# google-research/weatherbench2

Hardware: AMD Instinct MI355X
Metric: grid-point-evals/sec (721x1440x13) (higher is better)
Workload: dtype f32 (elementwise) + f64 (sums); 1 GPU; BASELINE configs[1]: 721x1440x13 f32, deterministic MSE+RMSE+MAE+Bias+ACC, 13 predefined slice regions, running init-time mean; pool_units=48, regions=13, rows_per_chunk=32, step=one wb2_det_suite_step call (K1 + K2 + time accumulate), parallelism=init-time shards x1, 1 all-reduce of [sum,count], launcher=single process

## Files before the change

### include/wb2hip.h

```cpp
#ifndef WB2HIP_H_
#define WB2HIP_H_

#include <stdint.h>

#ifdef __cplusplus
extern "C" {
#endif

#define WB2_VERSION 1

#define WB2_F32 0
#define WB2_F64 1

#define WB2_MODE_DET 0
#define WB2_MODE_DET_ACC 1
#define WB2_MODE_WIND 2

#define WB2_MODE_ENS 3

#define WB2_MODE_GAUSS 4
#define WB2_MODE_GAUSS_THR 5
#define WB2_MODE_SEEPS 7
#define WB2_MODE_ENS_THR 6

// ... 180 lines not shown

int wb2_ens_combine(int skipna, const double* partials, int64_t n_outer,
                    int32_t n_chunk, int32_t nwf, int32_t n_seg,
                    const int32_t* seg_eoff, int32_t n_ts,
                    const int32_t* band_chunk0, int32_t n_band,
                    const double* coef_band, const double* coef_seg,
                    const int32_t* region_wf, const double* region_wsum,
                    int32_t n_region, double* sums, double* metrics,
                    void* stream);

int wb2_time_accumulate(const double* values, int64_t n_lead, int64_t n_time,
                        int64_t n_tail, int skipna, double* sum, double* count,
                        void* stream);

int wb2_time_accumulate_scatter(int dtype, const void* values, int64_t n_lead,
                                int64_t n_time, int64_t n_tail, int skipna,
                                const int64_t* dst, double* sum, double* count,
                                void* stream);
int wb2_time_accumulate_runs(int dtype, const void* values, int64_t n_lead,
                             int64_t n_time, int64_t n_tail, int skipna,
                             const int64_t* dst, int64_t run, double* sum,
                             double* count, void* stream);

typedef struct wb2_plan_tables {
  int32_t n_row, n_col;
  int32_t n_chunk, n_ctile;
  int32_t n_seg, n_ts;
  int32_t n_band, n_region;
  const double* w_row;
  const double* w_col;
  const void* wfield;
  int32_t wfield_dtype;
  int32_t reserved;
  const double* aux;
  double scalar;
  const int32_t* chunk_row0;
  const int32_t* chunk_nrow;
  const int32_t* seg_col0;
  const int32_t* seg_eoff;
  const int32_t* band_chunk0;
  const double* coef_band;
  const double* coef_seg;
  const int32_t* region_wf;
  const double* region_wsum;
} wb2_plan_tables;

int wb2_det_suite_step(const wb2_plan_tables* plan, int mode, int dtype,
                       int skipna, const void* const* in,
                       const int64_t* const* slab, int aligned16,
                       int64_t n_outer, double* partials, double* metrics,
                       int64_t acc_lead, int64_t acc_time, int64_t acc_tail,
                       int acc_skipna, const int64_t* dst, double* sum,
                       double* count, void* stream);

int wb2_det_wind_suite_step(const wb2_plan_tables* plan, int mode, int dtype,
                            int skipna, const void* const* in,
                            const int64_t* const* slab, int aligned16,
                            int64_t n_outer, int64_t n_pair, double* partials,
                            double* wind_partials, double* metrics,
                            double* wind_metrics, void* stream);

int wb2_gather_accumulate(const double* arena, const int32_t* src,
                          const uint8_t* round32, int64_t n_out, int64_t n_time,
                          int skipna, const int64_t* sum_addr,
                          const int64_t* count_addr, void* stream);

int wb2_gather_accumulate_rows(const double* arena, const int32_t* src,
                               const uint8_t* round32, int64_t n_out,
                               int64_t n_time, int skipna,
                               const int64_t* sum_addr,
                               const int64_t* count_addr, const int64_t* rows,
                               const int32_t* sel, const int64_t* rsz8,
                               void* stream);

int wb2_program_create(void** program);
int wb2_program_destroy(void* program);
int wb2_program_add_launch(void* program, const wb2_plan_tables* plan, int mode,
                           int dtype, int skipna, int32_t n_in, int64_t n_outer,
                           int64_t n_pair, const int32_t* slot,
                           const int64_t* rel, double* partials,
                           double* wind_partials, int64_t arena_offset,
                           int side_stream);
int wb2_program_add_ens_launch(void* program, const wb2_plan_tables* plan,
                               int dtype, int skipna, int32_t n_member,
                               int64_t member_stride, int64_t n_outer,
                               const int32_t* slot, const int64_t* rel,
                               double* partials, int64_t arena_offset);
int wb2_program_add_gather(void* program, int32_t input, int64_t first,
                           int64_t count, int32_t source, int64_t step_bytes,
                           int32_t value_offset, const int32_t* cell,
                           const int64_t* base);
int wb2_program_add_sink(void* program, const int32_t* src,
                         const uint8_t* round32, int64_t n_out, int64_t n_time,
                         int skipna, const int32_t* sel, const int64_t* rsz8,
                         int64_t max_rows);
int wb2_program_finalize(void* program, double* arena, int32_t n_ptrs,
                         int32_t n_values);
int wb2_program_replay(void* program, const int64_t* ptrs, int32_t n_ptrs,
                       const int64_t* values, int32_t n_values,
                       const int64_t* sink_args, const int64_t* rows,
                       int32_t n_rows, void* stream);
int wb2_program_stats(void* program, double* seconds, int64_t* replays);

int wb2_energy_layout(int32_t n_member, int skipna, int has_wfield,
                      int32_t* block, int32_t* n_block, int32_t* n_slot);
int wb2_energy_score(int dtype, int skipna, const void* ens,
// ... 162 lines not shown
```

### weatherbench2_amd/_lib.py

```python
from __future__ import annotations

import ctypes
import os

import torch

from weatherbench2_amd import build as _build

WB2_F32, WB2_F64 = 0, 1
MODE_DET, MODE_DET_ACC, MODE_WIND, MODE_ENS, MODE_GAUSS = 0, 1, 2, 3, 4
MODE_GAUSS_THR, MODE_ENS_THR, MODE_SEEPS = 5, 6, 7
GENERIC_KQ = {MODE_GAUSS: 2, MODE_GAUSS_THR: 3, MODE_ENS_THR: 4,
              MODE_SEEPS: 1}
NMETRIC = 5
NMETRIC_ENS = 8
METRIC_INDEX = {'mse': 0, 'rmse': 1, 'mae': 2, 'bias': 3, 'acc': 4}
ENS_METRIC_INDEX = {'crps': 0, 'crps_spread': 1, 'crps_skill': 2,
                    'ensemble_mean_mse': 3, 'ensemble_mean_rmse': 4,
                    'ensemble_variance': 5, 'ensemble_stddev': 6,
                    'debiased_ensemble_mean_mse': 7}

_c = ctypes
_vp, _i32, _i64, _int = _c.c_void_p, _c.c_int32, _c.c_int64, _c.c_int
_u64 = _c.c_uint64



class PlanTables(_c.Structure):
  _fields_ = [
      ('n_row', _i32), ('n_col', _i32), ('n_chunk', _i32), ('n_ctile', _i32),
      ('n_seg', _i32), ('n_ts', _i32), ('n_band', _i32), ('n_region', _i32),
      ('w_row', _vp), ('w_col', _vp), ('wfield', _vp),
      ('wfield_dtype', _i32), ('reserved', _i32), ('aux', _vp),
      ('scalar', _c.c_double), ('chunk_row0', _vp), ('chunk_nrow', _vp),
      ('seg_col0', _vp), ('seg_eoff', _vp), ('band_chunk0', _vp),
      ('coef_band', _vp), ('coef_seg', _vp), ('region_wf', _vp),
      ('region_wsum', _vp)]


_SIGNATURES = {
    'wb2_version': (_int, []),
    'wb2_last_error': (_c.c_char_p, []),
    'wb2_num_slots': (_int, [_int, _int]),
    'wb2_tile_cols': (_int, [_int, _int, _int]),
    'wb2_tile_cols_ex': (_int, [_int, _int, _int, _int, _int, _int]),
    'wb2_stream_partials': (_int, [
        _int, _int, _int, _c.POINTER(_vp), _c.POINTER(_vp), _i64, _i32, _i32,
        _vp, _vp, _vp, _vp, _vp, _i32, _i32, _vp, _vp, _i32, _i32, _vp, _vp]),
    'wb2_stream_partials_ex': (_int, [
        _int, _int, _int, _c.POINTER(_vp), _c.POINTER(_vp), _i64, _i32, _i32,
        _vp, _vp, _vp, _int, _vp, _c.c_double, _vp, _vp, _i32, _i32, _vp, _vp,
        _i32, _i32, _vp, _vp]),
    'wb2_stream_partials_addr': (_int, [
        _int, _int, _int, _c.POINTER(_vp), _int, _i64, _i32, _i32,
        _vp, _vp, _vp, _int, _vp, _c.c_double, _vp, _vp, _i32, _i32, _vp, _vp,
        _i32, _i32, _vp, _vp]),
    'wb2_pairs_supported': (_int, [_int, _int, _int, _int, _int, _int]),
    'wb2_stream_partials_pairs': (_int, [
        _int, _int, _int, _c.POINTER(_vp), _c.POINTER(_vp), _int, _i64, _i64,
        _i32, _i32, _vp, _vp, _vp, _int, _vp, _vp, _i32, _i32, _vp, _vp, _i32,
        _i32, _vp, _vp, _vp]),
    'wb2_det_wind_suite_step': (_int, [
        _c.POINTER(PlanTables), _int, _int, _int, _c.POINTER(_vp),
        _c.POINTER(_vp), _int, _i64, _i64, _vp, _vp, _vp, _vp, _vp]),
    'wb2_det_combine': (_int, [
        _int, _int, _vp, _i64, _i32, _i32, _i32, _vp, _i32, _vp, _i32, _vp,
        _vp, _vp, _vp, _i32, _vp, _vp, _vp]),
    'wb2_det_suite_step': (_int, [
        _c.POINTER(PlanTables), _int, _int, _int, _c.POINTER(_vp),
        _c.POINTER(_vp), _int, _i64, _vp, _vp, _i64, _i64, _i64, _int, _vp,
        _vp, _vp, _vp]),
    'wb2_gather_accumulate': (_int, [_vp, _vp, _vp, _i64, _i64, _int, _vp, _vp,
                                     _vp]),
    'wb2_gather_accumulate_rows': (_int, [_vp, _vp, _vp, _i64, _i64, _int,
                                          _vp, _vp, _vp, _vp, _vp, _vp]),
    'wb2_program_create': (_int, [_c.POINTER(_vp)]),
    'wb2_program_destroy': (_int, [_vp]),
    'wb2_program_add_launch': (_int, [
        _vp, _c.POINTER(PlanTables), _int, _int, _int, _i32, _i64, _i64, _vp,
        _vp, _vp, _vp, _i64, _int]),
    'wb2_program_add_ens_launch': (_int, [
        _vp, _c.POINTER(PlanTables), _int, _int, _i32, _i64, _i64, _vp, _vp,
        _vp, _i64]),
    'wb2_program_add_gather': (_int, [_vp, _i32, _i64, _i64, _i32, _i64, _i32,
                                      _vp, _vp]),
    'wb2_program_add_sink': (_int, [_vp, _vp, _vp, _i64, _i64, _int, _vp, _vp,
                                    _i64]),
    'wb2_program_finalize': (_int, [_vp, _vp, _i32, _i32]),
    'wb2_program_replay': (_int, [_vp, _vp, _i32, _vp, _i32, _vp, _vp, _i32,
                                  _vp]),
    'wb2_program_stats': (_int, [_vp, _c.POINTER(_c.c_double),
                                 _c.POINTER(_i64)]),
    'wb2_energy_layout': (_int, [_i32, _int, _int, _c.POINTER(_i32),
                                 _c.POINTER(_i32), _c.POINTER(_i32)]),
    'wb2_energy_score': (_int, [
        _int, _int, _vp, _vp, _vp, _vp, _i32, _i64, _i64,
        _c.POINTER(PlanTables), _vp, _vp, _vp, _vp]),
    'wb2_time_accumulate': (_int, [_vp, _i64, _i64, _i64, _int, _vp, _vp,
                                   _vp]),
    'wb2_time_accumulate_scatter': (_int, [_int, _vp, _i64, _i64, _i64, _int,
                                           _vp, _vp, _vp, _vp]),
    'wb2_time_accumulate_runs': (_int, [_int, _vp, _i64, _i64, _i64, _int,
                                        _vp, _i64, _vp, _vp, _vp]),
    'wb2_ens_partials': (_int, [
        _int, _int, _vp, _vp, _vp, _vp, _i32, _i64, _i64, _i32, _i32, _vp, _vp,
        _vp, _vp, _vp, _i32, _i32, _vp, _vp, _i32, _i32, _vp, _vp]),
    'wb2_ens_partials_maps': (_int, [
        _int, _int, _vp, _vp, _vp, _vp, _i32, _i64, _i64, _i32, _i32, _vp, _vp,
        _vp, _vp, _vp, _i32, _i32, _vp, _vp, _i32, _i32, _vp, _vp, _vp]),
    'wb2_ens_partials_addr': (_int, [
        _int, _int, _vp, _vp, _i32, _i64, _i64, _i32, _i32, _vp, _vp, _vp, _vp,
        _vp, _i32, _i32, _vp, _vp, _i32, _i32, _vp, _vp]),
    'wb2_ens_partials_gather': (_int, [
        _int, _int, _vp, _vp, _vp, _i32, _i64, _i32, _i32, _vp, _vp, _vp, _vp,
        _vp, _i32, _i32, _vp, _vp, _i32, _i32, _vp, _vp, _vp]),
    'wb2_ens_threshold_partials': (_int, [
        _int, _int, _vp, _vp, _vp, _vp, _vp, _vp, _i32, _i64, _i64, _i32, _i32,
        _vp, _vp, _vp, _vp, _vp, _i32, _i32, _vp, _vp, _i32, _i32, _vp, _vp]),
    'wb2_ens_threshold_maps': (_int, [
        _int, _int, _vp, _vp, _vp, _vp, _vp, _vp, _i32, _i64, _i64, _i64, _vp,
        _vp]),
    'wb2_seeps_map': (_int, [_int, _c.POINTER(_vp), _c.POINTER(_vp), _i64, _i64,
                             _vp, _c.c_double, _vp, _vp]),
    'wb2_seeps_map_addr': (_int, [_int, _c.POINTER(_vp), _i64, _i64, _vp,
# ... 134 lines not shown
```

### weatherbench2_amd/csrc/stream_reduce.hip

```cpp

#include "common.hpp"
#include "trace.hpp"
#include "reduce_common.hpp"
#include "gauss_math.hpp"
#include "wb2hip.h"

#include <atomic>
#include <type_traits>

namespace wb2 {
namespace {

constexpr int kMaxIn = 4;

struct StreamParams {
  const void* in[kMaxIn];
  const long long* slab[kMaxIn];
  const double* w_row;
  const double* w_col;
  const void* wfield;
  const double* aux;
  double scalar;
  const int* chunk_row0;
  const int* chunk_nrow;
// ... 752 lines not shown
  } else {
#pragma clang loop unroll(disable)
    for (; r + U <= nrow; r += U, ++it)
      batch_v(std::integral_constant<int, U>{}, r, it & 1);
#pragma clang loop unroll(disable)
    for (; r < nrow; ++r, ++it)
      batch_v(std::integral_constant<int, 1>{}, r, it & 1);
  }

  if (p.w_col) {
#pragma unroll
    for (int e = 0; e < VEC; ++e) {
      const double wc = p.w_col[colb + e];
#pragma unroll
      for (int w = 0; w < NWF; ++w) {
#pragma unroll
        for (int k = 0; k < KD; ++k) acc[w][e][k] *= wc;
#pragma unroll
        for (int k = 0; k < KW; ++k) accw[w][e][k] *= wc;
      }
    }
  }
  fold_tile_to_segs<NWF, VEC, KD>(
      acc, lane, tile, colb, col0, p.n_col, p.seg_col0, p.seg_eoff, p.n_seg,
      p.n_ts,
      p.partials + (o * p.n_chunk + chunk) * (long long)(NWF * p.n_ts * KD));
  if (role == 1)
    fold_tile_to_segs<NWF, VEC, KW>(
        accw, lane, tile, colb, col0, p.n_col, p.seg_col0, p.seg_eoff, p.n_seg,
        p.n_ts,
        pp.wind_partials +
            (pair * p.n_chunk + chunk) * (long long)(NWF * p.n_ts * KW));
}

struct CombineParams {
  const double* partials;
  const int* seg_eoff;
  const int* band_chunk0;
  const double* coef_band;
  const double* coef_seg;
  const int* region_wf;
  const double* region_wsum;
  double* sums;
  double* metrics;
  long long n_outer;
  int n_chunk, nwf, n_seg, n_ts, n_band, n_region, K, mode, skipna;
  int group;
};

__device__ __forceinline__ double nan_if_zero(double d) {
  return d != 0.0 ? d : __builtin_nan("");
}

__device__ __forceinline__ void det_combine_body(const CombineParams& p,
                                                 const long long o,
                                                 double* lds) {
  const int K = p.K;
  const int cell = p.nwf * p.n_seg * K;
  double* bandsum = lds;
  double* rsum = lds + p.n_band * cell;
  const int tid = threadIdx.x;
  double* cseg = rsum + p.n_region * K * (1 + p.n_band);
  double* cband = cseg + p.n_region * p.n_seg;
  for (int i = tid; i < p.n_region * p.n_seg; i += blockDim.x)
    cseg[i] = p.coef_seg[i];
  for (int i = tid; i < p.n_region * p.n_band; i += blockDim.x)
    cband[i] = p.coef_band[i];
  const long long chunk_stride = (long long)p.nwf * p.n_ts * K;
  const double* part = p.partials + o * p.n_chunk * chunk_stride;

  if (p.group > 1) {
    const int G = p.group;
    for (int idx = tid; idx < p.n_band * cell * G; idx += blockDim.x) {
      const int ci = idx / G, g = idx - ci * G;
      const int b = ci / cell, j = ci - b * cell;
      const int w = j / (p.n_seg * K), sk = j - w * (p.n_seg * K);
      const int s = sk / K, k = sk - s * K;
      const int e0 = p.seg_eoff[s], ne = p.seg_eoff[s + 1] - e0;
      const int c0 = p.band_chunk0[b], n = (p.band_chunk0[b + 1] - c0) * ne;
      const double* base = part + ((long long)w * p.n_ts) * K + k +
                           c0 * chunk_stride + (long long)e0 * K;
      int c = g / ne, e = g - c * ne;
      const int dq = G / ne, dr = G - dq * ne;
      auto next = [&]() {
        const double* r = base + c * chunk_stride + (long long)e * K;
        c += dq;
        e += dr;
        if (e >= ne) {
          e -= ne;
          ++c;
        }
        return r;
      };
      double v = 0.0;
      int i = g;
      for (; i + 7 * G < n; i += 8 * G) {
        double t[8];
#pragma unroll
        for (int u = 0; u < 8; ++u) t[u] = *next();
#pragma unroll
        for (int u = 0; u < 8; ++u) v += t[u];
      }
      for (; i < n; i += G) v += *next();
      for (int off = G >> 1; off > 0; off >>= 1) v += __shfl_xor(v, off, kWave);
      if (g == 0) bandsum[ci] = v;
    }
  } else
  for (int idx = tid; idx < p.n_band * cell; idx += blockDim.x) {
    const int b = idx / cell, j = idx - b * cell;
    const int w = j / (p.n_seg * K), sk = j - w * (p.n_seg * K);
    const int s = sk / K, k = sk - s * K;
    const int e0 = p.seg_eoff[s], ne = p.seg_eoff[s + 1] - e0;
    const int c0 = p.band_chunk0[b], n = (p.band_chunk0[b + 1] - c0) * ne;
    const double* base = part + ((long long)w * p.n_ts) * K + k;
    const double* q = base + c0 * chunk_stride + (long long)e0 * K;
    const long long wrap = chunk_stride - (long long)ne * K;
    int e = 0;
    auto next = [&]() {
      const double* r = q;
      q += K;
      if (++e == ne) {
        e = 0;
        q += wrap;
      }
      return r;
    };
    double v = 0.0;
    int i = 0;
    for (; i + 32 <= n; i += 32) {
      double t[32];
#pragma unroll
      for (int u = 0; u < 32; ++u) t[u] = *next();
#pragma unroll
      for (int u = 0; u < 32; ++u) v += t[u];
    }
    for (; i + 16 <= n; i += 16) {
      double t[16];
#pragma unroll
      for (int u = 0; u < 16; ++u) t[u] = *next();
#pragma unroll
      for (int u = 0; u < 16; ++u) v += t[u];
    }
    for (; i + 4 <= n; i += 4) {
      double t[4];
#pragma unroll
      for (int u = 0; u < 4; ++u) t[u] = *next();
#pragma unroll
      for (int u = 0; u < 4; ++u) v += t[u];
    }
    for (; i < n; ++i) v += *next();
    bandsum[idx] = v;
  }
  __syncthreads();
  double* rb = rsum + p.n_region * K;
  for (int idx = tid; idx < p.n_region * p.n_band * K; idx += blockDim.x) {
    const int r = idx / (p.n_band * K), bk = idx - r * (p.n_band * K);
    const int b = bk / K, k = bk - b * K;
    const int wf = p.region_wf[r];
    const double cb = cband[r * p.n_band + b];
    double v = 0.0;
    if (cb != 0.0) {
      const double* row = bandsum + ((b * p.nwf + wf) * p.n_seg) * K + k;
      for (int s = 0; s < p.n_seg; ++s) {
        const double cs = cseg[r * p.n_seg + s];
        if (cs != 0.0) v += (cb * cs) * row[s * K];
      }
    }
    rb[idx] = v;
  }
  __syncthreads();
  for (int idx = tid; idx < p.n_region * K; idx += blockDim.x) {
    const int r = idx / K, k = idx - r * K;
    double v = 0.0;
    for (int b = 0; b < p.n_band; ++b)
      if (cband[r * p.n_band + b] != 0.0)
        v += rb[(r * p.n_band + b) * K + k];
    rsum[idx] = v;
    if (p.sums) p.sums[(o * p.n_region + r) * K + k] = v;
  }
  __syncthreads();
  if (!p.metrics) return;
  for (int r = tid; r < p.n_region; r += blockDim.x) {
    const double* s = rsum + r * K;
    const double nan = __builtin_nan("");
    const double wsum = nan_if_zero(p.region_wsum[r]);
    double mse = nan, rmse = nan, mae = nan, bias = nan, acc = nan;
    if (p.mode == WB2_MODE_ENS) {
      const double n_skill = p.skipna ? nan_if_zero(s[6]) : wsum;
      const double n_spread = p.skipna ? nan_if_zero(s[7]) : wsum;
      const double n_var = p.skipna ? nan_if_zero(s[8]) : wsum;
      const double n_deb = p.skipna ? nan_if_zero(s[9]) : wsum;
      const double skill = s[0] / n_skill, spread = s[1] / n_spread;
      const double emse = s[2] / n_skill, var = s[3] / n_var;
      const long long stride = (long long)p.n_region * p.n_outer;
      double* m = p.metrics + (long long)r * p.n_outer + o;
      m[WB2_ENS_CRPS * stride] = skill - 0.5 * spread;
      m[WB2_ENS_CRPS_SPREAD * stride] = spread;
      m[WB2_ENS_CRPS_SKILL * stride] = skill;
      m[WB2_ENS_MEAN_MSE * stride] = emse;
      m[WB2_ENS_MEAN_RMSE * stride] = sqrt(emse);
      m[WB2_ENS_VARIANCE * stride] = var;
      m[WB2_ENS_STDDEV * stride] = sqrt(s[4] / n_var);
      m[WB2_ENS_DEBIASED_MSE * stride] = s[5] / n_deb;
      continue;
    }
    if (p.mode >= WB2_MODE_GAUSS) {
      const int kq = p.skipna ? K / 2 : K;
      const long long stride = (long long)p.n_region * p.n_outer;
      double* m = p.metrics + (long long)r * p.n_outer + o;
      for (int i = 0; i < kq; ++i)
        m[i * stride] = s[i] / (p.skipna ? nan_if_zero(s[kq + i]) : wsum);
      continue;
    }
    if (p.mode == WB2_MODE_WIND) {
      const double den = p.skipna ? nan_if_zero(s[1]) : wsum;
      mse = s[0] / den;
      rmse = sqrt(mse);
    } else {
      const int kq = p.mode == WB2_MODE_DET_ACC ? 6 : 3;
      const double den_d = p.skipna ? nan_if_zero(s[kq]) : wsum;
      bias = s[0] / den_d;
      mae = s[1] / den_d;
      mse = s[2] / den_d;
      rmse = sqrt(mse);
      if (p.mode == WB2_MODE_DET_ACC) {
        const double den_p = p.skipna ? nan_if_zero(s[7]) : wsum;
        const double den_f = p.skipna ? nan_if_zero(s[8]) : wsum;
        const double den_t = p.skipna ? nan_if_zero(s[9]) : wsum;
        acc = (s[3] / den_p) / sqrt((s[4] / den_f) * (s[5] / den_t));
      }
    }
    const long long stride = (long long)p.n_region * p.n_outer;
    double* m = p.metrics + (long long)r * p.n_outer + o;
    m[WB2_METRIC_MSE * stride] = mse;
    m[WB2_METRIC_RMSE * stride] = rmse;
    m[WB2_METRIC_MAE * stride] = mae;
    m[WB2_METRIC_BIAS * stride] = bias;
    m[WB2_METRIC_ACC * stride] = acc;
  }
}

__global__ void __launch_bounds__(1024) det_combine_kernel(const CombineParams p) {
  extern __shared__ double lds[];
  det_combine_body(p, blockIdx.x, lds);
}

__global__ void __launch_bounds__(1024)
    det_combine2_kernel(const CombineParams a, const CombineParams b) {
  extern __shared__ double lds[];
  if ((long long)blockIdx.x < a.n_outer)
    det_combine_body(a, blockIdx.x, lds);
  else
    det_combine_body(b, (long long)blockIdx.x - a.n_outer, lds);
}

template <typename T>
__global__ void __launch_bounds__(256)
    time_accumulate_kernel(const T* __restrict__ values, long long n_lead,
                           long long n_time, long long n_tail, int skipna,
                           const long long* __restrict__ dst, long long run,
                           double* __restrict__ sum,
                           double* __restrict__ count) {
  const long long idx = (long long)blockIdx.x * blockDim.x + threadIdx.x;
  if (idx >= n_lead * n_tail) return;
  const long long l = idx / n_tail, j = idx - l * n_tail;
  long long out = idx;
  if (dst) {
    const long long r = run > 1 ? idx / run : idx;
    out = dst[r] + (idx - r * run);
  }
  double s = sum[out], c = count ? count[out] : 0.0;
  const T* base = values + l * n_time * n_tail + j;
  auto add = [&](double v) {
    const bool keep = !(skipna && is_nan(v));
    s += keep ? v : 0.0;
    c += keep ? 1.0 : 0.0;
  };
  long long t = 0;
  for (; t + 4 <= n_time; t += 4) {
    const T v0 = base[t * n_tail], v1 = base[(t + 1) * n_tail],
            v2 = base[(t + 2) * n_tail], v3 = base[(t + 3) * n_tail];
    add(v0);
    add(v1);
    add(v2);
    add(v3);
  }
  for (; t < n_time; ++t) add(base[t * n_tail]);
  sum[out] = s;
  if (count) count[out] = c;
}

__global__ void __launch_bounds__(256)
    gather_accumulate_kernel(const double* __restrict__ arena,
                             const int* __restrict__ src,
                             const unsigned char* __restrict__ round32,
                             long long n_out, long long n_time, int skipna,
                             const long long* __restrict__ sum_addr,
                             const long long* __restrict__ count_addr,
                             const long long* __restrict__ rows,
                             const int* __restrict__ sel,
                             const long long* __restrict__ rsz8) {
  const long long e = (long long)blockIdx.x * blockDim.x + threadIdx.x;
  if (e >= n_out) return;
  const long long shift = rows ? rows[sel[e]] * rsz8[e] : 0;
  double* sp = reinterpret_cast<double*>(sum_addr[e] + shift);
  double* cp = reinterpret_cast<double*>(count_addr[e] + shift);
  double s = *sp, c = *cp;
  const bool r32 = round32[e] != 0;
  const int* q = src + e * n_time;
  for (long long t = 0; t < n_time; ++t) {
    const int k = q[t];
    double v = k < 0 ? __builtin_nan("") : arena[k];
    if (r32) v = (double)(float)v;
    const bool keep = !(skipna && is_nan(v));
    s += keep ? v : 0.0;
    c += keep ? 1.0 : 0.0;
  }
  *sp = s;
  *cp = c;
}

template <typename T, int MODE>
constexpr bool field_f32_supported() {
  return std::is_same<T, float>::value &&
         (MODE == WB2_MODE_DET || MODE == WB2_MODE_DET_ACC ||
          MODE == WB2_MODE_WIND);
}
bool field_f32_supported(int dtype, int mode) {
  return dtype == WB2_F32 && (mode == WB2_MODE_DET || mode == WB2_MODE_DET_ACC ||
                              mode == WB2_MODE_WIND);
}

template <typename T, int VEC, int MODE, bool SKIPNA, bool WF>
int launch_stream(const StreamParams& p, int threads, hipStream_t stream) {
  const int nwave = threads / kWave;
  const int n_tblk = (p.n_ctile + nwave - 1) / nwave;
  const long long gy = p.n_outer < 32768 ? p.n_outer : 32768;
  const long long gz = (p.n_outer + gy - 1) / gy;
  const dim3 grid =
      (WF || MODE == WB2_MODE_SEEPS)
          ? dim3((unsigned)gy, (unsigned)(p.n_chunk * n_tblk), (unsigned)gz)
          : dim3((unsigned)(p.n_chunk * n_tblk), (unsigned)gy, (unsigned)gz);
// ... 678 lines not shown
                       static_cast<const double*>(values), (long long)n_lead,
                       (long long)n_time, (long long)n_tail, skipna, d,
                       (long long)run, sum, count);
  WB2_HIP_OK(hipGetLastError());
  return 0;
}

int wb2_det_suite_step(const wb2_plan_tables* plan, int mode, int dtype,
                       int skipna, const void* const* in,
                       const int64_t* const* slab, int aligned16,
                       int64_t n_outer, double* partials, double* metrics,
                       int64_t acc_lead, int64_t acc_time, int64_t acc_tail,
                       int acc_skipna, const int64_t* dst, double* sum,
                       double* count, void* stream) {
  WB2_TRACE();
  using namespace wb2;
  WB2_REQUIRE(plan != nullptr, "null plan");
  WB2_EMPTY_OK(n_outer);
  WB2_REQUIRE(in != nullptr || slab != nullptr, "null pointer argument");
  WB2_REQUIRE(metrics != nullptr, "metrics is null");
  const wb2_plan_tables& t = *plan;
  const int nm = mode >= WB2_MODE_GAUSS
                     ? (mode == WB2_MODE_GAUSS ? 2
                        : mode == WB2_MODE_GAUSS_THR ? 3
                        : mode == WB2_MODE_ENS_THR ? 4 : 1)
                     : WB2_NMETRIC;
  if (sum != nullptr || count != nullptr) {
    WB2_REQUIRE(sum && count, "sum and count go together");
    WB2_REQUIRE(acc_lead > 0 && acc_time > 0 && acc_tail > 0 &&
                    acc_lead * acc_time * acc_tail ==
                        (long long)nm * t.n_region * n_outer,
                "accumulate view [%lld][%lld][%lld] does not cover metrics "
                "[%d][%d][%lld]",
                (long long)acc_lead, (long long)acc_time, (long long)acc_tail,
                nm, t.n_region, (long long)n_outer);
  }
  int rc = stream_partials_impl(
      mode, dtype, skipna, in, slab, aligned16, n_outer, t.n_row, t.n_col,
      t.w_row, t.w_col, t.wfield, t.wfield_dtype, t.aux, t.scalar, t.chunk_row0,
      t.chunk_nrow, t.n_chunk, t.n_ctile, t.seg_col0, t.seg_eoff, t.n_seg,
      t.n_ts, partials, stream);
  if (rc != 0) return rc;
  rc = wb2_det_combine(mode, skipna, partials, n_outer, t.n_chunk,
                       t.wfield ? 2 : 1, t.n_seg, t.seg_eoff, t.n_ts,
                       t.band_chunk0, t.n_band, t.coef_band, t.coef_seg,
                       t.region_wf, t.region_wsum, t.n_region, nullptr, metrics,
                       stream);
  if (rc != 0 || sum == nullptr) return rc;
  return wb2_time_accumulate_scatter(WB2_F64, metrics, acc_lead, acc_time,
                                     acc_tail, acc_skipna, dst, sum, count,
                                     stream);
}

int wb2_det_wind_suite_step(const wb2_plan_tables* plan, int mode, int dtype,
                            int skipna, const void* const* in,
                            const int64_t* const* slab, int aligned16,
                            int64_t n_outer, int64_t n_pair, double* partials,
                            double* wind_partials, double* metrics,
                            double* wind_metrics, void* stream) {
  WB2_TRACE();
  using namespace wb2;
  WB2_REQUIRE(plan != nullptr, "null plan");
  WB2_EMPTY_OK(n_outer);
  WB2_REQUIRE(in != nullptr || slab != nullptr, "null pointer argument");
  WB2_REQUIRE(metrics != nullptr && (n_pair == 0 || wind_metrics != nullptr),
              "metrics is null");
  const wb2_plan_tables& t = *plan;
  int rc = stream_pairs_impl(mode, dtype, skipna, in, slab, aligned16, n_outer,
                             n_pair, t.n_row, t.n_col, t.w_row, t.w_col,
                             t.wfield, t.wfield_dtype, t.chunk_row0,
                             t.chunk_nrow, t.n_chunk, t.n_ctile, t.seg_col0,
                             t.seg_eoff, t.n_seg, t.n_ts, partials,
                             wind_partials, stream);
  if (rc != 0) return rc;
  return combine_det_and_wind(t, mode, skipna, partials, n_outer, wind_partials,
                              n_pair, metrics, wind_metrics, stream);
}

int wb2_gather_accumulate(const double* arena, const int32_t* src,
                          const uint8_t* round32, int64_t n_out, int64_t n_time,
                          int skipna, const int64_t* sum_addr,
                          const int64_t* count_addr, void* stream) {
  WB2_TRACE();
  using namespace wb2;
  WB2_EMPTY_OK(n_out);
  WB2_EMPTY_OK(n_time);
  WB2_REQUIRE(arena && src && round32 && sum_addr && count_addr,
              "null pointer argument");
  hipLaunchKernelGGL(gather_accumulate_kernel,
                     dim3((unsigned)((n_out + 255) / 256)), dim3(256), 0,
                     static_cast<hipStream_t>(stream), arena, src, round32,
                     (long long)n_out, (long long)n_time, skipna,
                     reinterpret_cast<const long long*>(sum_addr),
                     reinterpret_cast<const long long*>(count_addr),
                     (const long long*)nullptr, (const int*)nullptr,
                     (const long long*)nullptr);
  WB2_HIP_OK(hipGetLastError());
  return 0;
}

int wb2_gather_accumulate_rows(const double* arena, const int32_t* src,
                               const uint8_t* round32, int64_t n_out,
                               int64_t n_time, int skipna,
                               const int64_t* sum_addr,
                               const int64_t* count_addr, const int64_t* rows,
                               const int32_t* sel, const int64_t* rsz8,
// ... 88 lines not shown
```

### weatherbench2_amd/engine.py

```python
from __future__ import annotations

import os
import threading
import typing as t

import numpy as np
import torch

from weatherbench2_amd import _lib
from weatherbench2_amd.plan import ReductionPlan

_DTYPES = {torch.float32: _lib.WB2_F32, torch.float64: _lib.WB2_F64}
_FIELD_F32_MODES = (_lib.MODE_DET, _lib.MODE_DET_ACC, _lib.MODE_WIND)

_STAGED_UPLOAD_MIN_BYTES = 1 << 20

_LAUNCH_HOOK = None


def set_launch_hook(hook):
  global _LAUNCH_HOOK
  old, _LAUNCH_HOOK = _LAUNCH_HOOK, hook
  return old

# ... 340 lines not shown
      hook('begin', 'stream_partials')
    status = self._fn(
        self._tables_ref, self.mode, self.code, int(self.skipna),
        None if inputs is None else _lib.ptr_array(inputs),
        _lib.ptr_array(tables), int(self.aligned), self.n_outer, self.n_pair,
        self.partials.data_ptr(), self.wind_partials.data_ptr(),
        out.data_ptr(), out.data_ptr() + 8 * n_det,
        current_stream_ptr(dev) if stream_ptr is None else stream_ptr)
    if hook is not None:
      hook('end', 'stream_partials')
    if status != 0:
      _lib.check(status, 'wb2_det_wind_suite_step')
    flat = out.view(-1)
    return (flat[:n_det].view(_lib.NMETRIC, self.plan.n_region, self.n_outer),
            flat[n_det:n_det + _lib.NMETRIC * self.plan.n_region * self.n_pair]
            .view(_lib.NMETRIC, self.plan.n_region, self.n_pair))


class SuiteStep:

  def __init__(self, plan: ReductionPlan, mode: int, dtype: torch.dtype,
               skipna: bool, n_outer: int, aligned: bool = True,
               aux: t.Optional[torch.Tensor] = None, scalar: float = 0.0,
               by_address: bool = False):
    import ctypes
    lib = _lib.load()
    if dtype not in _DTYPES:
      raise TypeError(f'unsupported dtype {dtype}')
    self.lib, self.plan, self.mode, self.skipna = lib, plan, mode, bool(skipna)
    self.code, self.n_outer = _DTYPES[dtype], int(n_outer)
    self.by_address, self.aligned = bool(by_address), bool(aligned)
    dev = plan.device
    k = lib.wb2_num_slots(mode, int(skipna))
    field, field_code = plan.wfield, _lib.WB2_F64
    if (dtype == torch.float32 and mode in _FIELD_F32_MODES and
        getattr(plan, 'wfield32', None) is not None and
        os.environ.get('WB2HIP_FIELD_F32', '1') != '0'):
      field, field_code = plan.wfield32, _lib.WB2_F32
    aligned = aligned and (field is None or field.data_ptr() % 16 == 0)
    tile = lib.wb2_tile_cols_ex(mode, self.code, int(skipna),
                                int(plan.wfield is not None), plan.n_col,
                                int(aligned))
    self.tables, self._keep = plan_tables(plan, tile, field, field_code, aux,
                                          scalar)
    n_ts = self._keep[3]
    self.n_metric = _lib.GENERIC_KQ.get(mode, _lib.NMETRIC)
    self.partials = torch.empty((n_outer, plan.n_chunk, plan.nwf, n_ts, k),
                                dtype=torch.float64, device=dev)
    self.metrics = torch.empty((self.n_metric, plan.n_region, n_outer),
                               dtype=torch.float64, device=dev)
    self._tables_ref = ctypes.byref(self.tables)
    self._acc = (0, 0, 0, 0, None, None, None)
    self._acc_keep = None
    self._fn = lib.wb2_det_suite_step

  def accumulate_into(self, total: t.Optional[torch.Tensor],
                      count: t.Optional[torch.Tensor] = None,
                      view: t.Optional[tuple] = None, skipna: bool = False,
                      dst: t.Optional[torch.Tensor] = None) -> None:
    if total is None:
      self._acc, self._acc_keep = (0, 0, 0, 0, None, None, None), None
      return
    n_lead, n_time, n_tail = (int(v) for v in view)
    if n_lead * n_time * n_tail != self.metrics.numel():
      raise ValueError(f'view {view} does not cover the metrics '
                       f'{tuple(self.metrics.shape)}')
    for x in (total, count):
      if x.dtype != torch.float64 or not x.is_contiguous():
        raise ValueError('accumulators are contiguous float64 tensors')
    if dst is None and total.numel() != n_lead * n_tail:
      raise ValueError('accumulator shape mismatch')
    if dst is not None and (dst.dtype != torch.int64 or
                            dst.numel() != n_lead * n_tail):
      raise ValueError('dst is int64 with one entry per result element')
    self._acc = (n_lead, n_time, n_tail, int(skipna), _lib.ptr(dst) or None,
                 total.data_ptr(), count.data_ptr())
    self._acc_keep = (total, count, dst)

  def run(self, inputs: t.Optional[t.Sequence[torch.Tensor]],
          tables: t.Sequence[t.Optional[torch.Tensor]],
          metrics: t.Optional[torch.Tensor] = None,
          stream_ptr: t.Optional[int] = None) -> torch.Tensor:
    out = self.metrics if metrics is None else metrics
    if self.by_address != (inputs is None):
      raise ValueError('by_address steps take inputs=None and address tables')
    hook = _LAUNCH_HOOK
    if hook is not None:
      hook('begin', 'stream_partials')
    status = self._fn(
        self._tables_ref, self.mode, self.code, int(self.skipna),
        None if inputs is None else _lib.ptr_array(inputs),
        _lib.ptr_array(tables), int(self.aligned), self.n_outer,
        self.partials.data_ptr(), out.data_ptr(), *self._acc,
        current_stream_ptr(self.plan.device) if stream_ptr is None
        else stream_ptr)
    if hook is not None:
      hook('end', 'stream_partials')
    if status != 0:
      _lib.check(status, 'wb2_det_suite_step')
    return out

  def bind(self, inputs, tables, stream_ptr: t.Optional[int] = None):
    if self.by_address != (inputs is None):
      raise ValueError('by_address steps take inputs=None and address tables')
    fn = self._fn
    keep = (inputs, tables, self._acc_keep)
    args = (self._tables_ref, self.mode, self.code, int(self.skipna),
            None if inputs is None else _lib.ptr_array(inputs),
            _lib.ptr_array(tables), int(self.aligned), self.n_outer,
            self.partials.data_ptr(), self.metrics.data_ptr()) + self._acc + (
                current_stream_ptr(self.plan.device) if stream_ptr is None
                else stream_ptr,)

    def call(_keep=keep):
      if fn(*args) != 0:
        _lib.check(-1, 'wb2_det_suite_step')
    return call


GATHER_MAX_MEMBERS = {torch.float32: 128, torch.float64: 64}
_NAN_SLABS: dict = {}
_NAN_SLABS_LOCK = threading.Lock()


def nan_slab(device: torch.device, dtype: torch.dtype, n_elems: int):
  key = (str(device), dtype, int(n_elems))
  slab = _NAN_SLABS.get(key)
  if slab is None:
    with _NAN_SLABS_LOCK:
      slab = _NAN_SLABS.get(key)
      if slab is None:
        slab = torch.full((int(n_elems),), float('nan'), dtype=dtype,
                          device=device)
        if torch.device(device).type == 'cuda':
          torch.cuda.current_stream(device).synchronize()
        _NAN_SLABS[key] = slab
  return slab


def gather_pointers(base: torch.Tensor, index: np.ndarray, slab_elems: int):
  index = np.asarray(index, dtype=np.int64)
  ptrs = base.data_ptr() + index * (slab_elems * base.element_size())
  if (index < 0).any():
    hole = nan_slab(base.device, base.dtype, slab_elems).data_ptr()
    ptrs = np.where(index < 0, np.int64(hole), ptrs)
  return ptrs


def ensemble_reduce(plan: ReductionPlan, ens: torch.Tensor,
                    member_stride: int, n_member: int,
                    ens_slab: t.Optional[torch.Tensor], truth: torch.Tensor,
                    truth_slab: t.Optional[torch.Tensor], n_outer: int,
                    skipna: bool, want_sums: bool = False,
                    maps: t.Optional[torch.Tensor] = None,
                    member_ptrs: t.Optional[torch.Tensor] = None,
                    addresses: t.Optional[torch.Tensor] = None):
  lib = _lib.load()
  dev = plan.device
  dtype = ens.dtype
  if dtype not in _DTYPES or truth.dtype != dtype:
    raise TypeError(f'unsupported / mismatched dtypes {ens.dtype} {truth.dtype}')
  if addresses is not None:
    if (addresses.dtype != torch.int64 or addresses.device != dev or
        not addresses.is_contiguous() or addresses.numel() != 2 * n_outer or
        maps is not None or member_ptrs is not None):
      raise ValueError('addresses is a contiguous int64[2, n_outer] on the '
                       'plan device (no maps, no member_ptrs)')
  elif ens.device != dev or truth.device != dev or not truth.is_contiguous() or (
      not ens.is_contiguous() and ens_slab is None and member_ptrs is None):
# ... 787 lines not shown
```

Measured before the change: 509.1 billion grid-point-evals/s.

## Fuse combine and time-mean accumulation into one kernel with LDS-staged partials

Adds a fused det suite step whose combine kernel first stages each outer slice's partials and plan tables into LDS, then folds them into metrics. Where the accumulate view fits, a last-block-done ticket counter in a new workspace lets the final block for each tail index do the running time accumulation, removing the separate scatter kernel launch. The trade-off is large dynamic LDS per block (up to 160KB) with 1024-thread blocks, plus atomic publication of metrics and a dependence on counters being reset between calls.

```diff
diff --git a/include/wb2hip.h b/include/wb2hip.h
--- a/include/wb2hip.h
+++ b/include/wb2hip.h
@@ -256,6 +256,16 @@
                        int64_t acc_lead, int64_t acc_time, int64_t acc_tail,
                        int acc_skipna, const int64_t* dst, double* sum,
                        double* count, void* stream);
+
+int64_t wb2_det_suite_workspace_size(int64_t n_outer);
+int wb2_det_suite_step_fused(const wb2_plan_tables* plan, int mode, int dtype,
+                             int skipna, const void* const* in,
+                             const int64_t* const* slab, int aligned16,
+                             int64_t n_outer, double* partials,
+                             double* metrics, int64_t acc_lead,
+                             int64_t acc_time, int64_t acc_tail,
+                             int acc_skipna, const int64_t* dst, double* sum,
+                             double* count, void* workspace, void* stream);
 
 int wb2_det_wind_suite_step(const wb2_plan_tables* plan, int mode, int dtype,
                             int skipna, const void* const* in,
diff --git a/weatherbench2_amd/_lib.py b/weatherbench2_amd/_lib.py
--- a/weatherbench2_amd/_lib.py
+++ b/weatherbench2_amd/_lib.py
@@ -70,6 +70,11 @@
         _c.POINTER(PlanTables), _int, _int, _int, _c.POINTER(_vp),
         _c.POINTER(_vp), _int, _i64, _vp, _vp, _i64, _i64, _i64, _int, _vp,
         _vp, _vp, _vp]),
+    'wb2_det_suite_workspace_size': (_i64, [_i64]),
+    'wb2_det_suite_step_fused': (_int, [
+        _c.POINTER(PlanTables), _int, _int, _int, _c.POINTER(_vp),
+        _c.POINTER(_vp), _int, _i64, _vp, _vp, _i64, _i64, _i64, _int, _vp,
+        _vp, _vp, _vp, _vp]),
     'wb2_gather_accumulate': (_int, [_vp, _vp, _vp, _i64, _i64, _int, _vp, _vp,
                                      _vp]),
     'wb2_gather_accumulate_rows': (_int, [_vp, _vp, _vp, _i64, _i64, _int,
diff --git a/weatherbench2_amd/csrc/stream_reduce.hip b/weatherbench2_amd/csrc/stream_reduce.hip
--- a/weatherbench2_amd/csrc/stream_reduce.hip
+++ b/weatherbench2_amd/csrc/stream_reduce.hip
@@ -828,6 +828,23 @@
   return d != 0.0 ? d : __builtin_nan("");
 }
 
+struct FoldLds {
+  size_t coef_end, stage, total;
+};
+__host__ __device__ inline FoldLds fold_lds(int n_band, int nwf, int n_seg,
+                                            int n_region, int K, int n_chunk,
+                                            int n_ts) {
+  FoldLds l;
+  l.coef_end = (size_t)n_band * nwf * n_seg * K +
+               (size_t)n_region * K * (1 + (size_t)n_band) +
+               (size_t)n_region * ((size_t)n_seg + n_band);
+  const size_t n_int = (size_t)n_seg + 1 + (size_t)n_band + 1 + 1;
+  l.stage = (l.coef_end + (n_int + 1) / 2 + 1) & ~(size_t)1;
+  l.total = l.stage + (size_t)n_chunk * nwf * n_ts * K;
+  return l;
+}
+
+template <bool STAGED = false, bool PUBLISH = false>
 __device__ __forceinline__ void det_combine_body(const CombineParams& p,
                                                  const long long o,
                                                  double* lds) {
@@ -838,12 +855,83 @@
   const int tid = threadIdx.x;
   double* cseg = rsum + p.n_region * K * (1 + p.n_band);
   double* cband = cseg + p.n_region * p.n_seg;
-  for (int i = tid; i < p.n_region * p.n_seg; i += blockDim.x)
-    cseg[i] = p.coef_seg[i];
-  for (int i = tid; i < p.n_region * p.n_band; i += blockDim.x)
-    cband[i] = p.coef_band[i];
   const long long chunk_stride = (long long)p.nwf * p.n_ts * K;
   const double* part = p.partials + o * p.n_chunk * chunk_stride;
+  const int* seg_eoff = p.seg_eoff;
+  const int* band_chunk0 = p.band_chunk0;
+  if constexpr (STAGED) {
+    const int n_cs = p.n_region * p.n_seg, n_cb = p.n_region * p.n_band;
+    int* seg_l = reinterpret_cast<int*>(cband + n_cb);
+    int* band_l = seg_l + p.n_seg + 1;
+    double* stage =
+        lds + fold_lds(p.n_band, p.nwf, p.n_seg, p.n_region, K, p.n_chunk,
+                       p.n_ts).stage;
+    const double r_cs = p.coef_seg[min(tid, n_cs - 1)];
+    const double r_cb = p.coef_band[min(tid, n_cb - 1)];
+    const int r_se = p.seg_eoff[min(tid, p.n_seg)];
+    const int r_bc = p.band_chunk0[min(tid, p.n_band)];
+    const long long n = p.n_chunk * chunk_stride;
+    const double* src = part;
+    if ((reinterpret_cast<unsigned long long>(src) & 15) == 0 && (n & 1) == 0) {
+      const double2* src2 = reinterpret_cast<const double2*>(src);
+      double2* dst2 = reinterpret_cast<double2*>(stage);
+      const long long n2 = n >> 1;
+      for (long long i0 = tid; i0 - tid < n2; i0 += 4 * blockDim.x) {
+        double2 r[4];
+#pragma unroll
+        for (int u = 0; u < 4; ++u)
+          r[u] = src2[min(i0 + u * (long long)blockDim.x, n2 - 1)];
+#pragma unroll
+        for (int u = 0; u < 4; ++u) asm volatile("" ::"v"(r[u].x), "v"(r[u].y));
+#pragma unroll
+        for (int u = 0; u < 4; ++u) {
+          const long long i = i0 + u * (long long)blockDim.x;
+          if (i < n2) dst2[i] = r[u];
+        }
+      }
+    } else {
+      for (long long i0 = tid; i0 - tid < n; i0 += 8 * blockDim.x) {
+        double r[8];
+#pragma unroll
+        for (int u = 0; u < 8; ++u)
+          r[u] = src[min(i0 + u * (long long)blockDim.x, n - 1)];
+#pragma unroll
+        for (int u = 0; u < 8; ++u) asm volatile("" ::"v"(r[u]));
+#pragma unroll
+        for (int u = 0; u < 8; ++u) {
+          const long long i = i0 + u * (long long)blockDim.x;
+          if (i < n) stage[i] = r[u];
+        }
+      }
+    }
+    if (tid < n_cs) cseg[tid] = r_cs;
+    if (tid < n_cb) cband[tid] = r_cb;
+    if (tid <= p.n_seg) seg_l[tid] = r_se;
+    if (tid <= p.n_band) band_l[tid] = r_bc;
+    for (int i = tid + blockDim.x; i < n_cs; i += blockDim.x)
+      cseg[i] = p.coef_seg[i];
+    for (int i = tid + blockDim.x; i < n_cb; i += blockDim.x)
+      cband[i] = p.coef_band[i];
+    for (int i = tid + blockDim.x; i <= p.n_seg; i += blockDim.x)
+      seg_l[i] = p.seg_eoff[i];
+    for (int i = tid + blockDim.x; i <= p.n_band; i += blockDim.x)
+      band_l[i] = p.band_chunk0[i];
+    __syncthreads();
+    part = stage;
+    seg_eoff = seg_l;
+    band_chunk0 = band_l;
+  } else {
+    for (int i = tid; i < p.n_region * p.n_seg; i += blockDim.x)
+      cseg[i] = p.coef_seg[i];
+    for (int i = tid; i < p.n_region * p.n_band; i += blockDim.x)
+      cband[i] = p.coef_band[i];
+  }
+  auto put = [](double* at, double v) {
+    if constexpr (PUBLISH)
+      __hip_atomic_store(at, v, __ATOMIC_RELAXED, __HIP_MEMORY_SCOPE_AGENT);
+    else
+      *at = v;
+  };
 
   if (p.group > 1) {
     const int G = p.group;
@@ -852,8 +940,8 @@
       const int b = ci / cell, j = ci - b * cell;
       const int w = j / (p.n_seg * K), sk = j - w * (p.n_seg * K);
       const int s = sk / K, k = sk - s * K;
-      const int e0 = p.seg_eoff[s], ne = p.seg_eoff[s + 1] - e0;
-      const int c0 = p.band_chunk0[b], n = (p.band_chunk0[b + 1] - c0) * ne;
+      const int e0 = seg_eoff[s], ne = seg_eoff[s + 1] - e0;
+      const int c0 = band_chunk0[b], n = (band_chunk0[b + 1] - c0) * ne;
       const double* base = part + ((long long)w * p.n_ts) * K + k +
                            c0 * chunk_stride + (long long)e0 * K;
       int c = g / ne, e = g - c * ne;
@@ -886,8 +974,8 @@
     const int b = idx / cell, j = idx - b * cell;
     const int w = j / (p.n_seg * K), sk = j - w * (p.n_seg * K);
     const int s = sk / K, k = sk - s * K;
-    const int e0 = p.seg_eoff[s], ne = p.seg_eoff[s + 1] - e0;
-    const int c0 = p.band_chunk0[b], n = (p.band_chunk0[b + 1] - c0) * ne;
+    const int e0 = seg_eoff[s], ne = seg_eoff[s + 1] - e0;
+    const int c0 = band_chunk0[b], n = (band_chunk0[b + 1] - c0) * ne;
     const double* base = part + ((long long)w * p.n_ts) * K + k;
     const double* q = base + c0 * chunk_stride + (long long)e0 * K;
     const long long wrap = chunk_stride - (long long)ne * K;
@@ -970,14 +1058,14 @@
       const double emse = s[2] / n_skill, var = s[3] / n_var;
       const long long stride = (long long)p.n_region * p.n_outer;
       double* m = p.metrics + (long long)r * p.n_outer + o;
-      m[WB2_ENS_CRPS * stride] = skill - 0.5 * spread;
-      m[WB2_ENS_CRPS_SPREAD * stride] = spread;
-      m[WB2_ENS_CRPS_SKILL * stride] = skill;
-      m[WB2_ENS_MEAN_MSE * stride] = emse;
-      m[WB2_ENS_MEAN_RMSE * stride] = sqrt(emse);
-      m[WB2_ENS_VARIANCE * stride] = var;
-      m[WB2_ENS_STDDEV * stride] = sqrt(s[4] / n_var);
-      m[WB2_ENS_DEBIASED_MSE * stride] = s[5] / n_deb;
+      put(m + WB2_ENS_CRPS * stride, skill - 0.5 * spread);
+      put(m + WB2_ENS_CRPS_SPREAD * stride, spread);
+      put(m + WB2_ENS_CRPS_SKILL * stride, skill);
+      put(m + WB2_ENS_MEAN_MSE * stride, emse);
+      put(m + WB2_ENS_MEAN_RMSE * stride, sqrt(emse));
+      put(m + WB2_ENS_VARIANCE * stride, var);
+      put(m + WB2_ENS_STDDEV * stride, sqrt(s[4] / n_var));
+      put(m + WB2_ENS_DEBIASED_MSE * stride, s[5] / n_deb);
       continue;
     }
     if (p.mode >= WB2_MODE_GAUSS) {
@@ -985,7 +1073,7 @@
       const long long stride = (long long)p.n_region * p.n_outer;
       double* m = p.metrics + (long long)r * p.n_outer + o;
       for (int i = 0; i < kq; ++i)
-        m[i * stride] = s[i] / (p.skipna ? nan_if_zero(s[kq + i]) : wsum);
+        put(m + i * stride, s[i] / (p.skipna ? nan_if_zero(s[kq + i]) : wsum));
       continue;
     }
     if (p.mode == WB2_MODE_WIND) {
@@ -1008,11 +1096,11 @@
     }
     const long long stride = (long long)p.n_region * p.n_outer;
     double* m = p.metrics + (long long)r * p.n_outer + o;
-    m[WB2_METRIC_MSE * stride] = mse;
-    m[WB2_METRIC_RMSE * stride] = rmse;
-    m[WB2_METRIC_MAE * stride] = mae;
-    m[WB2_METRIC_BIAS * stride] = bias;
-    m[WB2_METRIC_ACC * stride] = acc;
+    put(m + WB2_METRIC_MSE * stride, mse);
+    put(m + WB2_METRIC_RMSE * stride, rmse);
+    put(m + WB2_METRIC_MAE * stride, mae);
+    put(m + WB2_METRIC_BIAS * stride, bias);
+    put(m + WB2_METRIC_ACC * stride, acc);
   }
 }
 
@@ -1064,6 +1152,80 @@
   for (; t < n_time; ++t) add(base[t * n_tail]);
   sum[out] = s;
   if (count) count[out] = c;
+}
+
+struct FoldTail {
+  double* sum;
+  double* count;
+  const long long* dst;
+  unsigned* counters;
+  long long acc_lead, acc_time, acc_tail;
+  int skipna;
+};
+
+template <bool TAIL>
+__global__ void __launch_bounds__(1024)
+    det_fold_mean_kernel(const CombineParams p, const FoldTail t) {
+  extern __shared__ double lds[];
+  const long long o = blockIdx.x;
+  det_combine_body<true, TAIL>(p, o, lds);
+  if constexpr (TAIL) {
+    const FoldLds l = fold_lds(p.n_band, p.nwf, p.n_seg, p.n_region, p.K,
+                               p.n_chunk, p.n_ts);
+    int* last = reinterpret_cast<int*>(lds + l.coef_end) + p.n_seg + 1 +
+                p.n_band + 1;
+    const long long j = o % t.acc_tail;
+    asm volatile("s_waitcnt vmcnt(0)" ::: "memory");
+    __syncthreads();
+    if (threadIdx.x == 0) {
+      const unsigned ticket = __hip_atomic_fetch_add(
+          t.counters + j, 1u, __ATOMIC_RELAXED, __HIP_MEMORY_SCOPE_AGENT);
+      const bool mine = ticket == (unsigned)(t.acc_time - 1);
+      if (mine) {
+        __hip_atomic_store(t.counters + j, 0u, __ATOMIC_RELAXED,
+                           __HIP_MEMORY_SCOPE_AGENT);
+        __builtin_amdgcn_fence(__ATOMIC_ACQUIRE, "agent");
+        asm volatile("s_waitcnt vmcnt(0)" ::: "memory");
+      }
+      *last = mine;
+    }
+    __syncthreads();
+    if (!*last) return;
+    const double* values = p.metrics;
+    for (long long lead = threadIdx.x; lead < t.acc_lead; lead += blockDim.x) {
+      const long long idx = lead * t.acc_tail + j;
+      const long long out = t.dst ? t.dst[idx] : idx;
+      double s = t.sum[out], c = t.count[out];
+      const double* base = values + lead * p.n_outer + j;
+      const int skipna = t.skipna;
+      auto add = [&](double v) {
+        const bool keep = !(skipna && is_nan(v));
+        s += keep ? v : 0.0;
+        c += keep ? 1.0 : 0.0;
+      };
+      long long ts = 0;
+      for (; ts + 16 <= t.acc_time; ts += 16) {
+        double v[16];
+#pragma unroll
+        for (int u = 0; u < 16; ++u) v[u] = base[(ts + u) * t.acc_tail];
+#pragma unroll
+        for (int u = 0; u < 16; ++u) add(v[u]);
+      }
+      for (; ts + 4 <= t.acc_time; ts += 4) {
+        const double v0 = base[ts * t.acc_tail],
+                     v1 = base[(ts + 1) * t.acc_tail],
+                     v2 = base[(ts + 2) * t.acc_tail],
+                     v3 = base[(ts + 3) * t.acc_tail];
+        add(v0);
+        add(v1);
+        add(v2);
+        add(v3);
+      }
+      for (; ts < t.acc_time; ++ts) add(base[ts * t.acc_tail]);
+      t.sum[out] = s;
+      t.count[out] = c;
+    }
+  }
 }
 
 __global__ void __launch_bounds__(256)
@@ -1848,6 +2010,107 @@
                                      stream);
 }
 
+int64_t wb2_det_suite_workspace_size(int64_t n_outer) {
+  return n_outer <= 0 ? 0 : (n_outer * (int64_t)sizeof(unsigned) + 15) / 16 * 16;
+}
+
+int wb2_det_suite_step_fused(const wb2_plan_tables* plan, int mode, int dtype,
+                             int skipna, const void* const* in,
+                             const int64_t* const* slab, int aligned16,
+                             int64_t n_outer, double* partials,
+                             double* metrics, int64_t acc_lead,
+                             int64_t acc_time, int64_t acc_tail,
+                             int acc_skipna, const int64_t* dst, double* sum,
+                             double* count, void* workspace, void* stream) {
+  WB2_TRACE();
+  using namespace wb2;
+  WB2_REQUIRE(plan != nullptr, "null plan");
+  WB2_EMPTY_OK(n_outer);
+  WB2_REQUIRE(in != nullptr || slab != nullptr, "null pointer argument");
+  WB2_REQUIRE(metrics != nullptr, "metrics is null");
+  WB2_REQUIRE(mode >= 0 && mode <= WB2_MODE_SEEPS, "unknown mode %d", mode);
+  const wb2_plan_tables& t = *plan;
+  const int nm = mode >= WB2_MODE_GAUSS
+                     ? (mode == WB2_MODE_GAUSS ? 2
+                        : mode == WB2_MODE_GAUSS_THR ? 3
+                        : mode == WB2_MODE_ENS_THR ? 4 : 1)
+                     : WB2_NMETRIC;
+  if (sum != nullptr || count != nullptr) {
+    WB2_REQUIRE(sum && count, "sum and count go together");
+    WB2_REQUIRE(workspace != nullptr, "accumulators need the workspace");
+    WB2_REQUIRE(acc_lead > 0 && acc_time > 0 && acc_tail > 0 &&
+                    acc_lead * acc_time * acc_tail ==
+                        (long long)nm * t.n_region * n_outer,
+                "accumulate view [%lld][%lld][%lld] does not cover metrics "
+                "[%d][%d][%lld]",
+                (long long)acc_lead, (long long)acc_time, (long long)acc_tail,
+                nm, t.n_region, (long long)n_outer);
+  }
+  const int nwf = t.wfield ? 2 : 1;
+  int rc = stream_partials_impl(
+      mode, dtype, skipna, in, slab, aligned16, n_outer, t.n_row, t.n_col,
+      t.w_row, t.w_col, t.wfield, t.wfield_dtype, t.aux, t.scalar, t.chunk_row0,
+      t.chunk_nrow, t.n_chunk, t.n_ctile, t.seg_col0, t.seg_eoff, t.n_seg,
+      t.n_ts, partials, stream);
+  if (rc != 0) return rc;
+  const int k = mode == WB2_MODE_ENS ? wb2_ens_num_slots(skipna)
+                                     : wb2_num_slots(mode, skipna);
+  const bool sane = t.seg_eoff && t.band_chunk0 && t.coef_band && t.coef_seg &&
+                    t.region_wf && t.region_wsum && partials && t.n_chunk > 0 &&
+                    t.n_ts >= t.n_seg && t.n_seg > 0 && t.n_band > 0 &&
+                    t.n_region > 0 && k > 0 && n_outer < (1ll << 31);
+  const size_t lds =
+      sane ? fold_lds(t.n_band, nwf, t.n_seg, t.n_region, k, t.n_chunk, t.n_ts)
+                     .total * sizeof(double)
+           : 0;
+  if (!sane || lds > 160 * 1024) {
+    rc = wb2_det_combine(mode, skipna, partials, n_outer, t.n_chunk, nwf,
+                         t.n_seg, t.seg_eoff, t.n_ts, t.band_chunk0, t.n_band,
+                         t.coef_band, t.coef_seg, t.region_wf, t.region_wsum,
+                         t.n_region, nullptr, metrics, stream);
+    if (rc != 0 || sum == nullptr) return rc;
+    return wb2_time_accumulate_scatter(WB2_F64, metrics, acc_lead, acc_time,
+                                       acc_tail, acc_skipna, dst, sum, count,
+                                       stream);
+  }
+  size_t unused = 0;
+  const CombineParams p = combine_params(
+      mode, skipna, k, partials, n_outer, t.n_chunk, nwf, t.n_seg, t.seg_eoff,
+      t.n_ts, t.band_chunk0, t.n_band, t.coef_band, t.coef_seg, t.region_wf,
+      t.region_wsum, t.n_region, nullptr, metrics, &unused);
+  const bool tail = sum != nullptr &&
+                    acc_lead == (long long)nm * t.n_region &&
+                    acc_time * acc_tail == n_outer;
+  FoldTail ft{};
+  if (tail) {
+    ft.sum = sum;
+    ft.count = count;
+    ft.dst = reinterpret_cast<const long long*>(dst);
+    ft.counters = static_cast<unsigned*>(workspace);
+    ft.acc_lead = acc_lead;
+    ft.acc_time = acc_time;
+    ft.acc_tail = acc_tail;
+    ft.skipna = acc_skipna;
+  }
+  auto* kernel = tail ? det_fold_mean_kernel<true> : det_fold_mean_kernel<false>;
+  if (lds > 64 * 1024) {
+    static std::atomic<bool> allowed[2];
+    if (!allowed[tail].load()) {
+      WB2_HIP_OK(hipFuncSetAttribute(
+          reinterpret_cast<const void*>(kernel),
+          hipFuncAttributeMaxDynamicSharedMemorySize, 160 * 1024));
+      allowed[tail].store(true);
+    }
+  }
+  hipLaunchKernelGGL(kernel, dim3((unsigned)n_outer), dim3(1024), lds,
+                     static_cast<hipStream_t>(stream), p, ft);
+  WB2_HIP_OK(hipGetLastError());
+  if (tail || sum == nullptr) return 0;
+  return wb2_time_accumulate_scatter(WB2_F64, metrics, acc_lead, acc_time,
+                                     acc_tail, acc_skipna, dst, sum, count,
+                                     stream);
+}
+
 int wb2_det_wind_suite_step(const wb2_plan_tables* plan, int mode, int dtype,
                             int skipna, const void* const* in,
                             const int64_t* const* slab, int aligned16,
diff --git a/weatherbench2_amd/engine.py b/weatherbench2_amd/engine.py
--- a/weatherbench2_amd/engine.py
+++ b/weatherbench2_amd/engine.py
@@ -416,7 +416,10 @@
     self._tables_ref = ctypes.byref(self.tables)
     self._acc = (0, 0, 0, 0, None, None, None)
     self._acc_keep = None
-    self._fn = lib.wb2_det_suite_step
+    self.workspace = torch.zeros(
+        (max(int(lib.wb2_det_suite_workspace_size(int(n_outer))), 16),),
+        dtype=torch.uint8, device=dev)
+    self._fn = lib.wb2_det_suite_step_fused
 
   def accumulate_into(self, total: t.Optional[torch.Tensor],
                       count: t.Optional[torch.Tensor] = None,
@@ -456,12 +459,13 @@
         None if inputs is None else _lib.ptr_array(inputs),
         _lib.ptr_array(tables), int(self.aligned), self.n_outer,
         self.partials.data_ptr(), out.data_ptr(), *self._acc,
+        self.workspace.data_ptr(),
         current_stream_ptr(self.plan.device) if stream_ptr is None
         else stream_ptr)
     if hook is not None:
       hook('end', 'stream_partials')
     if status != 0:
-      _lib.check(status, 'wb2_det_suite_step')
+      _lib.check(status, 'wb2_det_suite_step_fused')
     return out
 
   def bind(self, inputs, tables, stream_ptr: t.Optional[int] = None):
@@ -473,12 +477,13 @@
             None if inputs is None else _lib.ptr_array(inputs),
             _lib.ptr_array(tables), int(self.aligned), self.n_outer,
             self.partials.data_ptr(), self.metrics.data_ptr()) + self._acc + (
+                self.workspace.data_ptr(),
                 current_stream_ptr(self.plan.device) if stream_ptr is None
                 else stream_ptr,)
 
     def call(_keep=keep):
       if fn(*args) != 0:
-        _lib.check(-1, 'wb2_det_suite_step')
+        _lib.check(-1, 'wb2_det_suite_step_fused')
     return call
 
 
```

New measurement: 508.3 billion grid-point-evals/s (median of 2 runs). Within noise of the previous version (-0.2%).
